# reinterpretcat/qwen3-rs

Measured on AMD Instinct MI355X. Metric: decode tokens/sec Qwen3-0.6B Q8 g=64 @1 GPU; % of int8 HBM roofline, higher is better.
Workload: dtype i8 (int8 x int8 -> i32 group dots, f32 scales/accumulate); 1 GPU; qwen3-0.6b Q8 group=64 single-stream greedy decode, 8-token prompt, reference generate-mode call pattern (first forward at pos 7, zero KV prefix), ctx 3072, 2751 tokens; mode=reference summation order (bit-identical logits), replicas=1, checkpoint_seed=1234

## Files before the change

qwen3-rs_amd/csrc/q3_attn_short2.h:

```cpp
#if defined(__HIP_DEVICE_COMPILE__) && !defined(__gfx950__)
#error "k_attn_short2 relies on gfx950 s_barrier behaviour for terminated waves; validated on gfx950 only"
#endif
constexpr int kS2Threads = 512;
constexpr int kS2MaxT = 256;
__host__ __device__ inline size_t attn_short2_smem_bytes(int hd, int max_t) { return 4 * (size_t)max_t * (size_t)(hd + 4); }

template <int V> struct IntC { static constexpr int value = V; };

#ifdef Q3_DEV
#define ATT2_STAMP(i, thr) do { if (a.stamps != nullptr && (a.debug & 64) == 0 && blockIdx.x == 3 && (int)threadIdx.x == (thr)) a.stamps[i] = __builtin_amdgcn_s_memtime(); } while (0)
#else
#define ATT2_STAMP(i, thr) do { } while (0)
#endif

template <int HD>
__global__ __launch_bounds__(kS2Threads) void k_attn_short2(const AttnArgs a) {
    static_assert(HD == 128, "head dim instantiated");
    constexpr int NQ4 = HD / 4;
    constexpr int HALF = HD / 2;
    constexpr int LD = HD + 4;
    constexpr int VT = 64;
    extern __shared__ __attribute__((aligned(16))) float ptile[];
    float* const vtile = ptile + VT * LD;
    __shared__ __attribute__((aligned(16))) float q_s[HD];
    __shared__ __attribute__((aligned(16))) float sq_s[2 * HD];
    __shared__ __attribute__((aligned(16))) float att[kS2MaxT];
    __shared__ __attribute__((aligned(16))) float att_e[kS2MaxT];
    __shared__ __attribute__((aligned(16))) float att_p[kS2MaxT];
    __shared__ unsigned long long etab[32];
    __shared__ unsigned vflag;
    __shared__ unsigned bcount;
    ATT2_STAMP(0, 0);
    KSTAMP_BEGIN(a);
    Q3_PIN_S(a.st); Q3_PIN_S(a.pos_override); Q3_PIN_S(a.q); Q3_PIN_S(a.k_raw); Q3_PIN_S(a.key_cache); Q3_PIN_S(a.value_cache);
    Q3_PIN_S(a.q_norm_w); Q3_PIN_S(a.k_norm_w); Q3_PIN_S(a.rope); Q3_PIN_S(a.xb); Q3_PIN_S(a.n_heads); Q3_PIN_S(a.n_kv_heads);
    Q3_PIN_S(a.write_q);

    const int kv_mul = a.kv_mul, xq = (int)((blockIdx.x * a.kvh_magic) >> 20);
    const int kvh = (int)blockIdx.x - xq * a.n_kv_heads;
    const int h = kvh * kv_mul + xq;
    const int tid = threadIdx.x, lane = tid & 63;
    const int wave = __builtin_amdgcn_readfirstlane(tid >> 6);
    const size_t kvd = (size_t)a.n_kv_heads * HD;
    const int pos_v = a.pos_override >= 0 ? a.pos_override : a.st->pos;
    const float* kbase = a.key_cache + (size_t)kvh * HD;
    const float* vbase = a.value_cache + (size_t)kvh * HD;

    if (wave == 4 || wave == 5) {
        const int pos = __builtin_amdgcn_readfirstlane(pos_v);
        const int np = pos + 1;
        const bool vsplit = gridDim.y == 2 && np > 64;
        if (gridDim.y == 2 && blockIdx.y == 1 && np <= 64) return;
        if (vsplit && wave == 5) {
            __syncthreads();
            __syncthreads();
            if (np > 128) __syncthreads();
            __syncthreads();
            return;
        }
        const int e = vsplit ? 64 * (int)blockIdx.y + lane : 64 * (wave - 4) + lane;
        const unsigned eoff = 4u * (unsigned)e;
        float vv[kShortVSets][32];
        auto v_issue = [&](float (&R)[32], int c) {
#pragma unroll
            for (int u = 0; u < 32; ++u) R[u] = *(const float*)((const char*)(vbase + (size_t)min(32 * c + u, pos) * kvd) + eoff);
        };
        auto v_pull = [&](float (&R)[32], int c) {
            const float* vp = vtile + e;
#pragma unroll
            for (int u = 0; u < 32; ++u) R[u] = vp[min(32 * c + u, pos) * HD];
        };
        const bool vlds = np <= VT;
        if (tid == 256) { vflag = 0u; bcount = 0u; }
        if (!vlds) {
#pragma unroll
            for (int c = 0; c < 2; ++c) v_issue(vv[c], c);
        }
        __syncthreads();
        if (!vlds) {
#pragma unroll
            for (int c = 2; c < kShortVSets; ++c)
                if (32 * c < np) v_issue(vv[c], c);
        }
        __syncthreads();
        if (vlds) {
            while (__hip_atomic_load(&vflag, __ATOMIC_ACQUIRE, __HIP_MEMORY_SCOPE_WORKGROUP) < 4u) __builtin_amdgcn_s_sleep(1);
#pragma unroll
            for (int c = 0; c < VT / 32; ++c)
                if (32 * c < np) v_pull(vv[c], c);
        }
        if (np > 128) __syncthreads();
        __syncthreads();
        ATT2_STAMP(5, 256);
        const v4f e4 = ((const v4f*)att_e)[lane];
        float sum;
        if (np <= 128) {
            sum = seq_chain(-0.0f, (const v4f*)att_e, (((np + 3) >> 2) + 7) & ~7);
        } else {
            const float etot = (e4.x + e4.y) + (e4.z + e4.w);
            sum = spec_sum_lanes(etot, (np + 3) >> 2, [&](float s) { return chain4(s, e4); });
        }
        ATT2_STAMP(13, 256);
        const float inv = 1.0f / sum;
        v4f p4;
        p4.x = e4.x * inv; p4.y = e4.y * inv; p4.z = e4.z * inv; p4.w = e4.w * inv;
        ((v4f*)att_p)[lane] = p4;
        wave_lds_sync();
        float o = 0.0f;
        auto fold_chunk = [&](const float (&R)[32], int c) {
            const v4f* pp = (const v4f*)att_p + 8 * c;
            v4f pq[8];
#pragma unroll
            for (int u4 = 0; u4 < 8; ++u4) pq[u4] = pp[u4];
#pragma unroll
            for (int u4 = 0; u4 < 8; ++u4) {
                if (32 * c + 4 * u4 < np) {
                    const v4f pv = pq[u4];
                    const v2f t01 = (v2f){pv.x, pv.y} * (v2f){R[4 * u4 + 0], R[4 * u4 + 1]};
                    const v2f t23 = (v2f){pv.z, pv.w} * (v2f){R[4 * u4 + 2], R[4 * u4 + 3]};
                    o = o + t01.x;
                    o = o + t01.y;
                    o = o + t23.x;
                    o = o + t23.y;
                }
            }
        };
#pragma unroll
        for (int c = 0; c < kShortVSets; ++c)
            if (32 * c < np) fold_chunk(vv[c], c);
        for (int c = kShortVSets; 32 * c < np; c += 2) {
            v_issue(vv[0], c);
            if (32 * (c + 1) < np) v_issue(vv[1], c + 1);
            fold_chunk(vv[0], c);
            if (32 * (c + 1) < np) fold_chunk(vv[1], c + 1);
        }
        ATT2_STAMP(14, 256);
        a.xb[(size_t)h * HD + e] = o;
        if (a.xbq != nullptr) {
            const float m = group_max_f32(fabsf(o), a.xb_group);
            const float scale = m / 127.0f;
            const int qv = (scale != 0.0f) ? quant_round_i8(o / scale) : 0;
            const int idx = h * HD + e;
            a.xbq[idx] = (int8_t)qv;
            if ((idx & (a.xb_group - 1)) == 0) a.xbs[idx / a.xb_group] = scale;
        }
        ATT2_STAMP(6, 256);
        KSTAMP_END(a);
        return;
    }

    int pos, np;
    if (wave < 2) {
        const bool is_q = wave == 0;
        const float* rawp = is_q ? a.q + (size_t)h * HD : a.k_raw + (size_t)kvh * HD;
        const float r_lo = rawp[lane], r_hi = rawp[lane + HALF];
        const float* nw = is_q ? a.q_norm_w : a.k_norm_w;
        const float w_lo = nw[lane], w_hi = nw[lane + HALF];
        __builtin_amdgcn_sched_barrier(0);
        pos = __builtin_amdgcn_readfirstlane(pos_v);
        np = pos + 1;
        if (gridDim.y == 2 && blockIdx.y == 1 && np <= 64) return;
        const v2f cs = *(const v2f*)(a.rope + (size_t)pos * HD + 2 * lane);
        ATT2_STAMP(1, 0);
        float* sq = sq_s + (is_q ? 0 : HD);
        sq[lane] = r_lo * r_lo;
        sq[lane + HALF] = r_hi * r_hi;
        wave_lds_sync();
        const float ss = seq_chain(-0.0f, (const v4f*)sq, NQ4);
        const float f = 1.0f / sqrtf(ss / (float)HD + kEps);
        const float xv = w_lo * (f * r_lo);
        const float yv = w_hi * (f * r_hi);
        const float a0 = xv * cs.x, b0 = yv * cs.y;
        const float a1 = xv * cs.y, b1 = yv * cs.x;
        const float lo = a0 - b0, hi = a1 + b1;
        if (is_q) {
            q_s[lane] = lo;
            q_s[lane + HALF] = hi;
            if (a.write_q) {
                a.q[(size_t)h * HD + lane] = lo;
                a.q[(size_t)h * HD + lane + HALF] = hi;
            }
        } else if ((h % kv_mul) == 0 && blockIdx.y == 0) {
            float* krow = a.key_cache + (size_t)pos * kvd + (size_t)kvh * HD;
            krow[lane] = lo;
            krow[lane + HALF] = hi;
        }
        ATT2_STAMP(2, 0);
        __syncthreads();
        if (!is_q) {
            ptile[pos * LD + lane] = q_s[lane] * lo;
            ptile[pos * LD + lane + HALF] = q_s[lane + HALF] * hi;
        }
    } else {
        unsigned long long etv = 0ull;
        if (wave == 7 && lane < 32) etv = kExp2Tab[lane];
#ifdef Q3_DEV
        const int hint = a.row_steps;
#else
        constexpr int hint = 0;
#endif
        if (hint <= 0) {
            pos = __builtin_amdgcn_readfirstlane(pos_v);
            np = pos + 1;
            if (gridDim.y == 2 && blockIdx.y == 1 && np <= 64) return;
        }
        ATT2_STAMP(8, 128);
        const int sidx = 64 * ((wave & 1) + (wave >= 6 ? 2 : 0)) + lane;
        const int r0 = sidx >> 5, col = sidx & 31;
        const unsigned loff = 4u * ((unsigned)r0 * (unsigned)kvd + 4u * (unsigned)col);
        const int kmax = max(a.seq_len / 8 - 1, 0);
        float* lp = ptile + r0 * LD + 4 * col;
        float* lv = vtile + r0 * HD + 4 * col;
        auto stage = [&](auto tier, auto with_v) {
            constexpr int T = decltype(tier)::value;
            constexpr bool V = decltype(with_v)::value != 0;
            v4f rk[T], rv[V ? T : 1];
#pragma unroll
            for (int k = 0; k < T; ++k) rk[k] = *(const v4f*)((const char*)(kbase + (size_t)min(k, kmax) * 8 * kvd) + loff);
            __builtin_amdgcn_sched_barrier(0);
            if constexpr (V) {
#pragma unroll
                for (int k = 0; k < T; ++k) rv[k] = *(const v4f*)((const char*)(vbase + (size_t)min(k, kmax) * 8 * kvd) + loff);
            }
            ATT2_STAMP(9, 128);
            if (hint > 0) {
                pos = __builtin_amdgcn_readfirstlane(pos_v);
                np = pos + 1;
            }
            __syncthreads();
            const v4f qv = ((const v4f*)q_s)[col];
#pragma unroll
            for (int k = 0; k < T; ++k) {
                const v2f p01 = (v2f){qv.x, qv.y} * (v2f){rk[k].x, rk[k].y};
                const v2f p23 = (v2f){qv.z, qv.w} * (v2f){rk[k].z, rk[k].w};
                v4f pr; pr.x = p01.x; pr.y = p01.y; pr.z = p23.x; pr.w = p23.y;
                if (r0 + 8 * k < pos) *(v4f*)(lp + 8 * k * LD) = pr;
            }
            if (wave == 7 && lane < 32) etab[lane] = etv;
            ATT2_STAMP(11, 128);
            if constexpr (V) {
                __syncthreads();
#pragma unroll
                for (int k = 0; k < T; ++k)
                    if (r0 + 8 * k < np) *(v4f*)(lv + 8 * k * HD) = rv[k];
                __builtin_amdgcn_fence(__ATOMIC_RELEASE, "workgroup");
                if (lane == 0) __hip_atomic_fetch_add(&vflag, 1u, __ATOMIC_RELAXED, __HIP_MEMORY_SCOPE_WORKGROUP);
                ATT2_STAMP(10, 128);
            }
        };
        const int tn = hint > 0 ? hint : (pos + 8) >> 3;
        if (tn <= 1) stage(IntC<1>{}, IntC<1>{});
        else if (tn <= 2) stage(IntC<2>{}, IntC<1>{});
        else if (tn <= 3) stage(IntC<3>{}, IntC<1>{});
        else if (tn <= 4) stage(IntC<4>{}, IntC<1>{});
        else if (tn <= 6) stage(IntC<6>{}, IntC<1>{});
        else if (tn <= 8) stage(IntC<8>{}, IntC<1>{});
        else if (tn <= 12) stage(IntC<12>{}, IntC<0>{});
        else if (tn <= 16) stage(IntC<16>{}, IntC<0>{});
        else if (tn <= 24) stage(IntC<24>{}, IntC<0>{});
        else stage(IntC<32>{}, IntC<0>{});
        if (np <= VT) return;
        __syncthreads();
        if (wave >= 6 || np <= 128) return;
    }
    if (wave < 2) __syncthreads();
    ATT2_STAMP(3, 0);

    const int t = 64 * wave + lane;
    float sc = -__builtin_inff();
    if (64 * wave < np) {
        const float scale = 1.0f / sqrtf((float)HD);
        const v4f* pr = (const v4f*)(ptile + min(t, pos) * LD);
        float dot = -0.0f;
        v4f pa[8], pb[8];
#pragma unroll
        for (int u = 0; u < 8; ++u) pa[u] = pr[u];
#pragma unroll
        for (int b = 0; b < NQ4 / 8; ++b) {
            if (b + 1 < NQ4 / 8) {
#pragma unroll
                for (int u = 0; u < 8; ++u) pb[u] = pr[8 * (b + 1) + u];
                __builtin_amdgcn_s_waitcnt(0xC87F);
            } else {
                __builtin_amdgcn_s_waitcnt(0xC07F);
            }
            __builtin_amdgcn_sched_barrier(0);
#pragma unroll
            for (int u = 0; u < 8; ++u) dot = chain4(dot, pa[u]);
            __builtin_amdgcn_sched_barrier(0);
#pragma unroll
            for (int u = 0; u < 8; ++u) pa[u] = pb[u];
        }
        sc = t < np ? dot * scale : -__builtin_inff();
    }
    const bool one_wave = np <= 64;
    float m;
    if (!one_wave) {
        att[t] = sc;
        if (np <= 128) {
            att[t + 128] = -__builtin_inff();
            __builtin_amdgcn_fence(__ATOMIC_RELEASE, "workgroup");
            if (lane == 0) {
                __hip_atomic_fetch_add(&bcount, 1u, __ATOMIC_RELAXED, __HIP_MEMORY_SCOPE_WORKGROUP);
                while (__hip_atomic_load(&bcount, __ATOMIC_RELAXED, __HIP_MEMORY_SCOPE_WORKGROUP) < 2u) __builtin_amdgcn_s_sleep(1);
            }
            __builtin_amdgcn_fence(__ATOMIC_ACQUIRE, "workgroup");
        } else {
            __syncthreads();
        }
        ATT2_STAMP(4, 0);
        const v4f s4 = ((const v4f*)att)[lane];
        m = fmaxf(fmaxf(s4.x, s4.y), fmaxf(s4.z, s4.w));
    } else {
        ATT2_STAMP(4, 0);
        m = sc;
    }
    m = group_max_f32(m, 64);
    float ev = 0.0f;
    if (64 * wave < np) {
        ev = q3_expf_wave(t < np ? sc - m : 0.0f, etab);
        ev = t < np ? ev : 0.0f;
    }
    att_e[t] = ev;
    if (np <= 128) att_e[t + 128] = 0.0f;
    __syncthreads();
    KSTAMP_END(a);
}
```

Baseline: 1129 tokens/s.

## Stage V tile through LDS for split-V attention up to 128 positions

Extends the LDS-staged V path to split-V blocks with 65-128 positions. The staging waves (6,7) load the block's half-width V slice into a new LDS region and signal through vflag. The output waves then pull from LDS instead of issuing strided per-lane global loads. This restructures the output path into three compile-time variants, adds LDS traffic and a spin-wait, and only affects the first ~128 decode steps of a 2751-token run.

```diff
diff --git a/qwen3-rs_amd/csrc/q3_attn_short2.h b/qwen3-rs_amd/csrc/q3_attn_short2.h
--- a/qwen3-rs_amd/csrc/q3_attn_short2.h
+++ b/qwen3-rs_amd/csrc/q3_attn_short2.h
@@ -20,8 +20,10 @@
     constexpr int HALF = HD / 2;
     constexpr int LD = HD + 4;
     constexpr int VT = 64;
+    constexpr int VT2 = 128;
     extern __shared__ __attribute__((aligned(16))) float ptile[];
     float* const vtile = ptile + VT * LD;
+    float* const vhalf = ptile + VT2 * LD;
     __shared__ __attribute__((aligned(16))) float q_s[HD];
     __shared__ __attribute__((aligned(16))) float sq_s[2 * HD];
     __shared__ __attribute__((aligned(16))) float att[kS2MaxT];
@@ -60,7 +62,6 @@
         }
         const int e = vsplit ? 64 * (int)blockIdx.y + lane : 64 * (wave - 4) + lane;
         const unsigned eoff = 4u * (unsigned)e;
-        float vv[kShortVSets][32];
         auto v_issue = [&](float (&R)[32], int c) {
 #pragma unroll
             for (int u = 0; u < 32; ++u) R[u] = *(const float*)((const char*)(vbase + (size_t)min(32 * c + u, pos) * kvd) + eoff);
@@ -70,82 +71,106 @@
 #pragma unroll
             for (int u = 0; u < 32; ++u) R[u] = vp[min(32 * c + u, pos) * HD];
         };
+        auto v_pull_half = [&](float (&R)[32], int c) {
+            const float* vp = vhalf + lane;
+#pragma unroll
+            for (int u = 0; u < 32; ++u) R[u] = vp[min(32 * c + u, pos) * (HD / 2)];
+        };
         const bool vlds = np <= VT;
+        const bool vlds2 = vsplit && np <= VT2;
         if (tid == 256) { vflag = 0u; bcount = 0u; }
-        if (!vlds) {
-#pragma unroll
-            for (int c = 0; c < 2; ++c) v_issue(vv[c], c);
-        }
-        __syncthreads();
-        if (!vlds) {
-#pragma unroll
-            for (int c = 2; c < kShortVSets; ++c)
-                if (32 * c < np) v_issue(vv[c], c);
-        }
-        __syncthreads();
-        if (vlds) {
-            while (__hip_atomic_load(&vflag, __ATOMIC_ACQUIRE, __HIP_MEMORY_SCOPE_WORKGROUP) < 4u) __builtin_amdgcn_s_sleep(1);
-#pragma unroll
-            for (int c = 0; c < VT / 32; ++c)
-                if (32 * c < np) v_pull(vv[c], c);
-        }
-        if (np > 128) __syncthreads();
-        __syncthreads();
-        ATT2_STAMP(5, 256);
-        const v4f e4 = ((const v4f*)att_e)[lane];
-        float sum;
-        if (np <= 128) {
-            sum = seq_chain(-0.0f, (const v4f*)att_e, (((np + 3) >> 2) + 7) & ~7);
-        } else {
-            const float etot = (e4.x + e4.y) + (e4.z + e4.w);
-            sum = spec_sum_lanes(etot, (np + 3) >> 2, [&](float s) { return chain4(s, e4); });
-        }
-        ATT2_STAMP(13, 256);
-        const float inv = 1.0f / sum;
-        v4f p4;
-        p4.x = e4.x * inv; p4.y = e4.y * inv; p4.z = e4.z * inv; p4.w = e4.w * inv;
-        ((v4f*)att_p)[lane] = p4;
-        wave_lds_sync();
-        float o = 0.0f;
-        auto fold_chunk = [&](const float (&R)[32], int c) {
-            const v4f* pp = (const v4f*)att_p + 8 * c;
-            v4f pq[8];
-#pragma unroll
-            for (int u4 = 0; u4 < 8; ++u4) pq[u4] = pp[u4];
-#pragma unroll
-            for (int u4 = 0; u4 < 8; ++u4) {
-                if (32 * c + 4 * u4 < np) {
-                    const v4f pv = pq[u4];
-                    const v2f t01 = (v2f){pv.x, pv.y} * (v2f){R[4 * u4 + 0], R[4 * u4 + 1]};
-                    const v2f t23 = (v2f){pv.z, pv.w} * (v2f){R[4 * u4 + 2], R[4 * u4 + 3]};
-                    o = o + t01.x;
-                    o = o + t01.y;
-                    o = o + t23.x;
-                    o = o + t23.y;
+        auto out = [&](auto road_c) {
+            constexpr int ROAD = decltype(road_c)::value;
+            constexpr int NSETS = ROAD == 0 ? VT / 32 : ROAD == 1 ? VT2 / 32 : kShortVSets;
+            float vv[NSETS][32];
+            if constexpr (ROAD == 2) {
+#pragma unroll
+                for (int c = 0; c < 2; ++c) v_issue(vv[c], c);
+            }
+            __syncthreads();
+            if constexpr (ROAD == 2) {
+#pragma unroll
+                for (int c = 2; c < kShortVSets; ++c)
+                    if (32 * c < np) v_issue(vv[c], c);
+            }
+            ATT2_STAMP(12, 256);
+            __syncthreads();
+            ATT2_STAMP(15, 256);
+            if constexpr (ROAD == 0) {
+                while (__hip_atomic_load(&vflag, __ATOMIC_ACQUIRE, __HIP_MEMORY_SCOPE_WORKGROUP) < 4u) __builtin_amdgcn_s_sleep(1);
+#pragma unroll
+                for (int c = 0; c < NSETS; ++c)
+                    if (32 * c < np) v_pull(vv[c], c);
+            }
+            if constexpr (ROAD == 1) {
+                while (__hip_atomic_load(&vflag, __ATOMIC_ACQUIRE, __HIP_MEMORY_SCOPE_WORKGROUP) < 2u) __builtin_amdgcn_s_sleep(1);
+#pragma unroll
+                for (int c = 0; c < NSETS; ++c)
+                    if (32 * c < np) v_pull_half(vv[c], c);
+            }
+            if (ROAD == 2 && np > 128) __syncthreads();
+            __syncthreads();
+            ATT2_STAMP(5, 256);
+            const v4f e4 = ((const v4f*)att_e)[lane];
+            float sum;
+            if (ROAD != 2 || np <= 128) {
+                sum = seq_chain(-0.0f, (const v4f*)att_e, (((np + 3) >> 2) + 7) & ~7);
+            } else {
+                const float etot = (e4.x + e4.y) + (e4.z + e4.w);
+                sum = spec_sum_lanes(etot, (np + 3) >> 2, [&](float s) { return chain4(s, e4); });
+            }
+            ATT2_STAMP(13, 256);
+            const float inv = 1.0f / sum;
+            v4f p4;
+            p4.x = e4.x * inv; p4.y = e4.y * inv; p4.z = e4.z * inv; p4.w = e4.w * inv;
+            ((v4f*)att_p)[lane] = p4;
+            wave_lds_sync();
+            float o = 0.0f;
+            auto fold_chunk = [&](const float (&R)[32], int c) {
+                const v4f* pp = (const v4f*)att_p + 8 * c;
+                v4f pq[8];
+#pragma unroll
+                for (int u4 = 0; u4 < 8; ++u4) pq[u4] = pp[u4];
+#pragma unroll
+                for (int u4 = 0; u4 < 8; ++u4) {
+                    if (32 * c + 4 * u4 < np) {
+                        const v4f pv = pq[u4];
+                        const v2f t01 = (v2f){pv.x, pv.y} * (v2f){R[4 * u4 + 0], R[4 * u4 + 1]};
+                        const v2f t23 = (v2f){pv.z, pv.w} * (v2f){R[4 * u4 + 2], R[4 * u4 + 3]};
+                        o = o + t01.x;
+                        o = o + t01.y;
+                        o = o + t23.x;
+                        o = o + t23.y;
+                    }
                 }
-            }
-        };
-#pragma unroll
-        for (int c = 0; c < kShortVSets; ++c)
-            if (32 * c < np) fold_chunk(vv[c], c);
-        for (int c = kShortVSets; 32 * c < np; c += 2) {
-            v_issue(vv[0], c);
-            if (32 * (c + 1) < np) v_issue(vv[1], c + 1);
-            fold_chunk(vv[0], c);
-            if (32 * (c + 1) < np) fold_chunk(vv[1], c + 1);
-        }
-        ATT2_STAMP(14, 256);
-        a.xb[(size_t)h * HD + e] = o;
-        if (a.xbq != nullptr) {
-            const float m = group_max_f32(fabsf(o), a.xb_group);
-            const float scale = m / 127.0f;
-            const int qv = (scale != 0.0f) ? quant_round_i8(o / scale) : 0;
-            const int idx = h * HD + e;
-            a.xbq[idx] = (int8_t)qv;
-            if ((idx & (a.xb_group - 1)) == 0) a.xbs[idx / a.xb_group] = scale;
-        }
-        ATT2_STAMP(6, 256);
-        KSTAMP_END(a);
+            };
+#pragma unroll
+            for (int c = 0; c < NSETS; ++c)
+                if (32 * c < np) fold_chunk(vv[c], c);
+            if constexpr (ROAD == 2) {
+                for (int c = kShortVSets; 32 * c < np; c += 2) {
+                    v_issue(vv[0], c);
+                    if (32 * (c + 1) < np) v_issue(vv[1], c + 1);
+                    fold_chunk(vv[0], c);
+                    if (32 * (c + 1) < np) fold_chunk(vv[1], c + 1);
+                }
+            }
+            ATT2_STAMP(14, 256);
+            a.xb[(size_t)h * HD + e] = o;
+            if (a.xbq != nullptr) {
+                const float m = group_max_f32(fabsf(o), a.xb_group);
+                const float scale = m / 127.0f;
+                const int qv = (scale != 0.0f) ? quant_round_i8(o / scale) : 0;
+                const int idx = h * HD + e;
+                a.xbq[idx] = (int8_t)qv;
+                if ((idx & (a.xb_group - 1)) == 0) a.xbs[idx / a.xb_group] = scale;
+            }
+            ATT2_STAMP(6, 256);
+            KSTAMP_END(a);
+        };
+        if (vlds) out(IntC<0>{});
+        else if (vlds2) out(IntC<1>{});
+        else out(IntC<2>{});
         return;
     }
 
@@ -213,8 +238,9 @@
         float* lv = vtile + r0 * HD + 4 * col;
         auto stage = [&](auto tier, auto with_v) {
             constexpr int T = decltype(tier)::value;
-            constexpr bool V = decltype(with_v)::value != 0;
-            v4f rk[T], rv[V ? T : 1];
+            constexpr bool V = decltype(with_v)::value == 1;
+            constexpr bool V2 = decltype(with_v)::value == 2;
+            v4f rk[T], rv[V || V2 ? T : 1];
 #pragma unroll
             for (int k = 0; k < T; ++k) rk[k] = *(const v4f*)((const char*)(kbase + (size_t)min(k, kmax) * 8 * kvd) + loff);
             __builtin_amdgcn_sched_barrier(0);
@@ -229,6 +255,14 @@
             }
             __syncthreads();
             const v4f qv = ((const v4f*)q_s)[col];
+            if constexpr (V2) {
+                const int vrow = 4 * (wave & 1) + (lane >> 4);
+                const unsigned vcol = 4u * (64u * blockIdx.y + 4u * (unsigned)(lane & 15));
+#pragma unroll
+                for (int k = 0; k < T; ++k)
+                    rv[k] = *(const v4f*)((const char*)vbase + (4u * (unsigned)min(vrow + 8 * k, pos) * (unsigned)kvd + vcol));
+                __builtin_amdgcn_sched_barrier(0);
+            }
 #pragma unroll
             for (int k = 0; k < T; ++k) {
                 const v2f p01 = (v2f){qv.x, qv.y} * (v2f){rk[k].x, rk[k].y};
@@ -247,19 +281,31 @@
                 if (lane == 0) __hip_atomic_fetch_add(&vflag, 1u, __ATOMIC_RELAXED, __HIP_MEMORY_SCOPE_WORKGROUP);
                 ATT2_STAMP(10, 128);
             }
+            if constexpr (V2) {
+                __syncthreads();
+                const int vrow = 4 * (wave & 1) + (lane >> 4);
+                float* lh = vhalf + vrow * (HD / 2) + 4 * (lane & 15);
+#pragma unroll
+                for (int k = 0; k < T; ++k)
+                    if (vrow + 8 * k < np) *(v4f*)(lh + 8 * k * (HD / 2)) = rv[k];
+                __builtin_amdgcn_fence(__ATOMIC_RELEASE, "workgroup");
+                if (lane == 0) __hip_atomic_fetch_add(&vflag, 1u, __ATOMIC_RELAXED, __HIP_MEMORY_SCOPE_WORKGROUP);
+                ATT2_STAMP(10, 384);
+            }
         };
         const int tn = hint > 0 ? hint : (pos + 8) >> 3;
+        const bool v2 = hint <= 0 && wave >= 6 && gridDim.y == 2;
         if (tn <= 1) stage(IntC<1>{}, IntC<1>{});
         else if (tn <= 2) stage(IntC<2>{}, IntC<1>{});
         else if (tn <= 3) stage(IntC<3>{}, IntC<1>{});
         else if (tn <= 4) stage(IntC<4>{}, IntC<1>{});
         else if (tn <= 6) stage(IntC<6>{}, IntC<1>{});
         else if (tn <= 8) stage(IntC<8>{}, IntC<1>{});
-        else if (tn <= 12) stage(IntC<12>{}, IntC<0>{});
-        else if (tn <= 16) stage(IntC<16>{}, IntC<0>{});
+        else if (tn <= 12) { if (v2) stage(IntC<12>{}, IntC<2>{}); else stage(IntC<12>{}, IntC<0>{}); }
+        else if (tn <= 16) { if (v2) stage(IntC<16>{}, IntC<2>{}); else stage(IntC<16>{}, IntC<0>{}); }
         else if (tn <= 24) stage(IntC<24>{}, IntC<0>{});
         else stage(IntC<32>{}, IntC<0>{});
-        if (np <= VT) return;
+        if (np <= VT || (v2 && np <= VT2)) return;
         __syncthreads();
         if (wave >= 6 || np <= 128) return;
     }
```

Result: no change. 1127 tokens/s (median of 2 runs) (-0.2%).
